# ratschlab/SVGP-VAE

Hardware: AMD Instinct MI355X
Metric: SVGPVAE train steps/sec, rotated MNIST (N=4050, M=32, L=16) (higher is better)
Workload: dtype f64; 1 GPU; BASELINE configs[1]: rotated-MNIST SVGPVAE_Hensman, m=32 inducing, L=16, GPLVM dim 8, batch 256 per GPU, N_train=4050, GECO + clip_qs, float64; global_batch=256, rows_per_gpu=256, launch=eager phases (faster of hipGraph replay / eager phases in an untimed probe), parallelism=dp1, single_stat_block=0

## Files before the change

svgp-vae_amd/csrc/vae_dev.hpp:

```cpp
#pragma once
#include "common.hpp"

namespace svgp_vae {

#define VAE_NT 512
#define VAE_SCRATCH 4096

typedef double d4v_t __attribute__((ext_vector_type(4)));

template <int NTAP, bool TW, bool ELU_BIAS, int CI, int CO, int NT = VAE_NT>
__device__ __forceinline__ void gg_fwd(const real* in, int Hi, int Wi, int Hs, int Ws, int sy, int sx,
                                       const int (&oy)[NTAP], const int (&ox)[NTAP], const int (&woff)[NTAP],
                                       const real* W, int ldw, const real* bias, real* out, int Wo, int osy, int osx,
                                       int ooy, int oox) {
    constexpr int KQ = (CI + 3) / 4;
    const int lane = threadIdx.x & 63, wave = threadIdx.x >> 6, nwave = NT >> 6, r = lane & 15, q = lane >> 4;
    const int NP = Hs * Ws, ngrp = (NP + 15) >> 4;
    real breg[NTAP * KQ];
#pragma unroll
    for (int t = 0; t < NTAP; ++t)
#pragma unroll
        for (int kq = 0; kq < KQ; ++kq) {
            const int c = kq * 4 + q, cc = c < CI ? c : CI - 1, rc = r < CO ? r : CO - 1;
            const real v = W[woff[t] + (TW ? rc * ldw + cc : cc * ldw + rc)];
// ... 96 lines not shown
    static __device__ void fwd(const real* in, const real* w, const real* bias, real* out) {
        if constexpr (CIN == 1) {
            for (int it = threadIdx.x; it < NPIX * COUT; it += NT) {
                const int co = it % COUT, p = it / COUT, y = p / HOUT, x = p % HOUT;
                real acc = bias[co];
#pragma unroll
                for (int ky = 0; ky < 3; ++ky)
#pragma unroll
                    for (int kx = 0; kx < 3; ++kx) acc += in[(2 * y + ky) * HS + 2 * x + kx] * w[(ky * 3 + kx) * COUT + co];
                out[it] = elu_f(acc);
            }
            return;
        }
        const int oy[9] = {0, 0, 0, 1, 1, 1, 2, 2, 2}, ox[9] = {0, 1, 2, 0, 1, 2, 0, 1, 2};
        int wo[9];
#pragma unroll
        for (int t = 0; t < 9; ++t) wo[t] = t * CIN * COUT;
        gg_fwd<9, false, true, CIN, COUT, NT>(in, HS, HS, HOUT, HOUT, 2, 2, oy, ox, wo, w, COUT, bias, out, HOUT, 1, 1, 0, 0);
    }

    static __device__ void bwd_data(const real* dpre, const real* w, real* din) {
        {
            const int oy[4] = {0, 0, -1, -1}, ox[4] = {0, -1, 0, -1};
            const int wo[4] = {(0 * 3 + 0) * CIN * COUT, (0 * 3 + 2) * CIN * COUT, (2 * 3 + 0) * CIN * COUT, (2 * 3 + 2) * CIN * COUT};
            gg_fwd<4, true, false, COUT, CIN, NT>(dpre, HOUT, HOUT, (HS + 1) / 2, (HS + 1) / 2, 1, 1, oy, ox, wo, w, COUT, nullptr,
                                              din, HS, 2, 2, 0, 0);
        }
        {
            const int oy[2] = {0, -1}, ox[2] = {0, 0};
            const int wo[2] = {(0 * 3 + 1) * CIN * COUT, (2 * 3 + 1) * CIN * COUT};
            gg_fwd<2, true, false, COUT, CIN, NT>(dpre, HOUT, HOUT, (HS + 1) / 2, HS / 2, 1, 1, oy, ox, wo, w, COUT, nullptr, din,
                                              HS, 2, 2, 0, 1);
        }
        {
            const int oy[2] = {0, 0}, ox[2] = {0, -1};
            const int wo[2] = {(1 * 3 + 0) * CIN * COUT, (1 * 3 + 2) * CIN * COUT};
            gg_fwd<2, true, false, COUT, CIN, NT>(dpre, HOUT, HOUT, HS / 2, (HS + 1) / 2, 1, 1, oy, ox, wo, w, COUT, nullptr, din,
                                              HS, 2, 2, 1, 0);
        }
        {
            const int oy[1] = {0}, ox[1] = {0};
            const int wo[1] = {(1 * 3 + 1) * CIN * COUT};
            gg_fwd<1, true, false, COUT, CIN, NT>(dpre, HOUT, HOUT, HS / 2, HS / 2, 1, 1, oy, ox, wo, w, COUT, nullptr, din, HS, 2,
                                              2, 1, 1);
        }
    }

    static __device__ void bwd_weight(const real* in, const real* dpre, real* gw, real* gb, real* scratch) {
        if constexpr (CIN == 1) {
            constexpr int NO = 9 * COUT, NCH = NT / NO;
            static_assert(NCH >= 1 && NO * NCH <= VAE_SCRATCH, "chunk layout");
            const int o = threadIdx.x % NO, ch = threadIdx.x / NO, t = o / COUT, co = o % COUT, ky = t / 3, kx = t % 3;
            if (ch < NCH) {
                real acc = 0;
                for (int p = ch; p < NPIX; p += NCH) {
                    const int y = p / HOUT, x = p % HOUT;
                    acc += in[(2 * y + ky) * HS + 2 * x + kx] * dpre[p * COUT + co];
                }
                scratch[ch * NO + o] = acc;
            }
            __syncthreads();
            if (threadIdx.x < NO) {
                real tsum = 0;
#pragma unroll
                for (int c = 0; c < NCH; ++c) tsum += scratch[c * NO + threadIdx.x];
                gw[threadIdx.x] += tsum;
            }
            __syncthreads();
        } else {
            auto tapfn = [](int t) { return TapP{t / 3, t % 3, t * CIN * COUT, 0, 0}; };
            gg_wgrad<9, CIN, COUT, NT>(in, HS, HS, HOUT, HOUT, 2, 2, tapfn, dpre, HOUT, 1, 1, gw);
        }
        bias_grad<NPIX, COUT, NT>(dpre, gb, scratch);
    }
};

template <int HS, int PAD, int CIN, int COUT, int NT = VAE_NT>
struct UpConv3 {
    static constexpr int HOUT = 2 * HS - 2 + 2 * PAD;
    static constexpr int NPIX = HOUT * HOUT;
    static constexpr int NWE = 16 * CIN * COUT;
    static constexpr int NW = 9 * CIN * COUT;
    static constexpr int COG = (COUT % 2 == 0) ? 2 : 1;
    static constexpr int NCG = COUT / COG;
    static constexpr int CIG = (CIN % 2 == 0) ? 2 : 1;
    static constexpr int NIG = CIN / CIG;
    static __device__ __forceinline__ int T(int pi, int k) { return (k + pi >= 2) ? 1 : 0; }

    static __device__ void build_weff(const real* w, real* We) {
        for (int e = threadIdx.x; e < NWE; e += NT) {
            const int co = e % COUT, ci = (e / COUT) % CIN, tap = (e / (COUT * CIN)) % 4, cls = e / (COUT * CIN * 4);
            const int ty = tap >> 1, tx = tap & 1, py = cls >> 1, px = cls & 1;
            real s = 0;
#pragma unroll
            for (int ky = 0; ky < 3; ++ky)
#pragma unroll
                for (int kx = 0; kx < 3; ++kx)
                    if (T(py, ky) == ty && T(px, kx) == tx) s += w[((ky * 3 + kx) * CIN + ci) * COUT + co];
            We[e] = s;
        }
    }
    static __device__ void fold_grad(const real* gWe, real* gw) {
        for (int e = threadIdx.x; e < NW; e += NT) {
            const int co = e % COUT, ci = (e / COUT) % CIN, kx = (e / (COUT * CIN)) % 3, ky = e / (COUT * CIN * 3);
            real s = 0;
#pragma unroll
            for (int py = 0; py < 2; ++py)
#pragma unroll
                for (int px = 0; px < 2; ++px)
                    s += gWe[(((py * 2 + px) * 4 + T(py, ky) * 2 + T(px, kx)) * CIN + ci) * COUT + co];
            gw[e] = s;
        }
    }

    template <bool ROLL = false>
    static __device__ void fwd_valu(const real* in, const real* We, const real* bias, real* out) {
        constexpr int TAP_UNROLL = ROLL ? 1 : 2;
        for (int it = threadIdx.x; it < NPIX * NCG; it += NT) {
            const int cg = it % NCG, p = it / NCG, x = p % HOUT, y = p / HOUT;
            const int by = y - PAD, bx = x - PAD, py = by & 1, px = bx & 1, Y = by >> 1, X = bx >> 1;
            real acc[COG];
#pragma unroll
            for (int g = 0; g < COG; ++g) acc[g] = bias[cg * COG + g];
            const real* wc = We + ((py * 2 + px) * 4) * CIN * COUT + cg * COG;
#pragma unroll TAP_UNROLL
            for (int ty = 0; ty < 2; ++ty) {
                const int sy = Y + ty;
                const bool vy = (unsigned)sy < (unsigned)HS;
#pragma unroll TAP_UNROLL
                for (int tx = 0; tx < 2; ++tx) {
                    const int sx = X + tx;
                    const bool valid = vy && ((unsigned)sx < (unsigned)HS);
                    const real* src = in + (valid ? (sy * HS + sx) * CIN : 0);
                    const real* wk = wc + (ty * 2 + tx) * CIN * COUT;
#pragma unroll
                    for (int ci = 0; ci < CIN; ++ci) {
                        const real a = valid ? src[ci] : real(0);
#pragma unroll
                        for (int g = 0; g < COG; ++g) acc[g] += a * wk[ci * COUT + g];
                    }
                }
            }
#pragma unroll
            for (int g = 0; g < COG; ++g) out[p * COUT + cg * COG + g] = elu_f(acc[g]);
        }
    }

    static __device__ void bwd_data_valu(const real* dpre, const real* We, real* din) {
        for (int it = threadIdx.x; it < HS * HS * NIG; it += NT) {
            const int ig = it % NIG, ps = it / NIG, Xs = ps % HS, Ys = ps / HS;
            real acc[CIG];
#pragma unroll
            for (int g = 0; g < CIG; ++g) acc[g] = 0;
#pragma unroll 1
            for (int cy = 0; cy < 4; ++cy) {
                const int py = cy >> 1, ty = cy & 1;
                const int y = 2 * (Ys - ty) + py + PAD;
                const bool vy = (unsigned)y < (unsigned)HOUT;
#pragma unroll
                for (int cx = 0; cx < 4; ++cx) {
                    const int px = cx >> 1, tx = cx & 1;
                    const int x = 2 * (Xs - tx) + px + PAD;
                    const bool valid = vy && ((unsigned)x < (unsigned)HOUT);
                    const real* dp = dpre + (valid ? (y * HOUT + x) * COUT : 0);
                    const real* wk = We + (((py * 2 + px) * 4 + ty * 2 + tx) * CIN + ig * CIG) * COUT;
#pragma unroll
                    for (int co = 0; co < COUT; ++co) {
                        const real d = valid ? dp[co] : real(0);
#pragma unroll
                        for (int g = 0; g < CIG; ++g) acc[g] += d * wk[g * COUT + co];
                    }
                }
            }
#pragma unroll
            for (int g = 0; g < CIG; ++g) din[ps * CIN + ig * CIG + g] = acc[g];
        }
    }

    static __device__ void bwd_weight_valu(const real* in, const real* dpre, real* gWe, real* gb, real* scratch) {
        constexpr int NTC = 16 * CIN;
        constexpr int NCH0 = NT / NTC, NCH1 = VAE_SCRATCH / NWE;
        constexpr int NCH = NCH0 < NCH1 ? (NCH0 < 1 ? 1 : NCH0) : NCH1;
        constexpr int NG = HS + 1;
        const int tc = threadIdx.x % NTC, chunk = threadIdx.x / NTC;
        if (chunk < NCH) {
            const int ci = tc % CIN, tap = (tc / CIN) % 4, cls = tc / (CIN * 4);
            const int ty = tap >> 1, tx = tap & 1, py = cls >> 1, px = cls & 1;
            real acc[COUT];
#pragma unroll
            for (int co = 0; co < COUT; ++co) acc[co] = 0;
#pragma unroll 2
            for (int idx = chunk; idx < NG * NG; idx += NCH) {
                const int Y = idx / NG - 1, X = idx % NG - 1;
                const int y = 2 * Y + py + PAD, x = 2 * X + px + PAD, sy = Y + ty, sx = X + tx;
                const bool valid = ((unsigned)y < (unsigned)HOUT) && ((unsigned)x < (unsigned)HOUT) &&
                                   ((unsigned)sy < (unsigned)HS) && ((unsigned)sx < (unsigned)HS);
                const real a = valid ? in[(sy * HS + sx) * CIN + ci] : real(0);
                const real* dp = dpre + (valid ? (y * HOUT + x) * COUT : 0);
#pragma unroll
                for (int co = 0; co < COUT; ++co) acc[co] += a * dp[co];
            }
#pragma unroll
            for (int co = 0; co < COUT; ++co) scratch[chunk * NWE + tc * COUT + co] = acc[co];
        }
        __syncthreads();
        for (int widx = threadIdx.x; widx < NWE; widx += NT) {
            real s = 0;
#pragma unroll
            for (int c = 0; c < NCH; ++c) s += scratch[c * NWE + widx];
            gWe[widx] += s;
        }
        __syncthreads();
        constexpr int BCH = 32;
        if (threadIdx.x < BCH * COUT) {
            const int co = threadIdx.x % COUT, chunk2 = threadIdx.x / COUT;
            real s = 0;
            for (int p = chunk2; p < NPIX; p += BCH) s += dpre[p * COUT + co];
            scratch[threadIdx.x] = s;
        }
        __syncthreads();
        if (threadIdx.x < COUT) {
            real t = 0;
#pragma unroll
            for (int c = 0; c < BCH; ++c) t += scratch[c * COUT + threadIdx.x];
            gb[threadIdx.x] += t;
        }
        __syncthreads();
    }

    static __device__ void bwd_data_mfma(const real* dpre, const real* We, real* din) {
        int oy[16], ox[16], wo[16];
#pragma unroll
        for (int t = 0; t < 16; ++t) {
            const int py = (t >> 3) & 1, ty = (t >> 2) & 1, px = (t >> 1) & 1, tx = t & 1;
            oy[t] = py + PAD - 2 * ty;
            ox[t] = px + PAD - 2 * tx;
            wo[t] = ((py * 2 + px) * 4 + ty * 2 + tx) * CIN * COUT;
        }
        gg_fwd<16, true, false, COUT, CIN, NT>(dpre, HOUT, HOUT, HS, HS, 2, 2, oy, ox, wo, We, COUT, nullptr, din, HS, 1, 1, 0, 0);
    }

    static __device__ void bwd_weight_mfma(const real* in, const real* dpre, real* gWe, real* gb, real* scratch) {
        if (COUT >= 2) {
            auto tapfn = [](int t) {
                const int opy = (t >> 3) & 1, opx = (t >> 2) & 1, ty = (t >> 1) & 1, tx = t & 1;
                const int by = opy - PAD, bx = opx - PAD, py = by & 1, px = bx & 1;
                return TapP{(by - py) / 2 + ty, (bx - px) / 2 + tx, ((py * 2 + px) * 4 + ty * 2 + tx) * CIN * COUT, opy, opx};
            };
            gg_wgrad<16, CIN, COUT, NT>(in, HS, HS, HOUT / 2, HOUT / 2, 1, 1, tapfn, dpre, HOUT, 2, 2, gWe);
        } else {
            constexpr int NCH = NT / 16;
            constexpr int NG = HS + 1;
            const int ct = threadIdx.x & 15, chunk = threadIdx.x >> 4;
            const int cls = ct >> 2, tap = ct & 3, ty = tap >> 1, tx = tap & 1, py = cls >> 1, px = cls & 1;
            real acc[CIN];
#pragma unroll
            for (int ci = 0; ci < CIN; ++ci) acc[ci] = 0;
            for (int idx = chunk; idx < NG * NG; idx += NCH) {
                const int Y = idx / NG - 1, X = idx % NG - 1;
                const int y = 2 * Y + py + PAD, x = 2 * X + px + PAD, sy = Y + ty, sx = X + tx;
                const bool valid = ((unsigned)y < (unsigned)HOUT) && ((unsigned)x < (unsigned)HOUT) &&
                                   ((unsigned)sy < (unsigned)HS) && ((unsigned)sx < (unsigned)HS);
                const real d = valid ? dpre[y * HOUT + x] : real(0);
                const real* ip = in + (valid ? (sy * HS + sx) * CIN : 0);
#pragma unroll
                for (int ci = 0; ci < CIN; ++ci) acc[ci] += ip[ci] * d;
            }
#pragma unroll
            for (int ci = 0; ci < CIN; ++ci) scratch[chunk * (16 * CIN) + ct * CIN + ci] = acc[ci];
            __syncthreads();
            for (int widx = threadIdx.x; widx < 16 * CIN; widx += NT) {
                real s = 0;
#pragma unroll 8
                for (int c = 0; c < NCH; ++c) s += scratch[c * (16 * CIN) + widx];
                gWe[widx] += s;
            }
        }
        __syncthreads();
        bias_grad<NPIX, COUT, NT>(dpre, gb, scratch);
    }
};

template <int NT> using UpC1T = UpConv3<4, 1, 8, 8, NT>;
using UpC1 = UpC1T<VAE_NT>;
template <int NT> using UpC2T = UpConv3<8, 0, 8, 8, NT>;
using UpC2 = UpC2T<VAE_NT>;
template <int NT> using UpC3T = UpConv3<14, 1, 8, 1, NT>;
using UpC3 = UpC3T<VAE_NT>;
#define DEC_NWE 2176
static_assert(UpC1::NWE + UpC2::NWE + UpC3::NWE == DEC_NWE, "effective weights of the three up-convolutions");

using EncC1 = Conv3<28, 1, 0, 2, 1, 8, 13>;
using EncC2 = Conv3<13, 1, 0, 2, 8, 8, 6>;
using EncC3 = Conv3<6, 1, 0, 2, 8, 8, 2>;

__device__ __forceinline__ void lds_copy_in(real* dst, const real* __restrict__ src, int n) {
    for (int i = threadIdx.x; i < n; i += blockDim.x) dst[i] = src[i];
}
__device__ __forceinline__ void lds_copy_out(real* __restrict__ dst, const real* src, int n) {
    for (int i = threadIdx.x; i < n; i += blockDim.x) dst[i] = src[i];
}
__device__ __forceinline__ void lds_zero(real* dst, int n) {
    for (int i = threadIdx.x; i < n; i += blockDim.x) dst[i] = 0;
}

struct EncOff { int c1w, c1b, c2w, c2b, c3w, c3b, dw, db, n; };
struct DecOff { int dw, db, c1w, c1b, c2w, c2b, c3w, c3b, n; };

__device__ __host__ inline EncOff enc_off(int L) {
    EncOff o; int p = 0;
    o.c1w = p; p += 72; o.c1b = p; p += 8; o.c2w = p; p += 576; o.c2b = p; p += 8;
    o.c3w = p; p += 576; o.c3b = p; p += 8; o.dw = p; p += 32 * 2 * L; o.db = p; p += 2 * L; o.n = p;
    return o;
}
__device__ __host__ inline DecOff dec_off(int L) {
    DecOff o; int p = 0;
    o.dw = p; p += L * 128; o.db = p; p += 128; o.c1w = p; p += 576; o.c1b = p; p += 8;
    o.c2w = p; p += 576; o.c2b = p; p += 8; o.c3w = p; p += 72; o.c3b = p; p += 1; o.n = p;
    return o;
}


struct DecWgradArgs {
    int b, L, geco, n_slots, n_types;
    real inv_bglobal;
    const real* state; const real* images; const real* z; const real* h0; const real* a1; const real* a2; const real* recon;
    const real* d2; const real* d1; const real* dh0;
    real* part;
};
__host__ __device__ constexpr int dec_wgrad_mask(int n_types, int ty) { return n_types == 1 ? 7 : n_types == 2 ? (ty == 0 ? 1 : 6) : (1 << ty); }
__host__ __device__ constexpr int dec_wgrad_lds_mask(int nt, int L, int mask) {
    return ((mask & 1) ? 1568 + 784 + 128 : 0) + ((mask & 2) ? 512 + 1568 + 1024 : 0) +
           ((mask & 4) ? 128 + 512 + 128 + 64 + 1024 + L * 128 + 128 : 0) + 32 + ((mask & 3) ? (nt <= 256 ? 2048 : 4096) : 256);
}
__host__ __device__ constexpr int dec_wgrad_lds(int nt, int L, int n_types) {
    int mx = 0;
    for (int ty = 0; ty < n_types; ++ty) {
        const int v = dec_wgrad_lds_mask(nt, L, dec_wgrad_mask(n_types, ty));
        mx = v > mx ? v : mx;
    }
    return mx;
}

template <int NT>
__device__ __forceinline__ void decoder_wgrad_rider(const DecWgradArgs& a, int rider, real* smem) {
    static_assert(NT >= 256 && NT <= 512, "bias / chunk layouts are sized for 256..512 threads");
    const DecOff od = dec_off(a.L);
    const int tyo = rider / a.n_slots, slot = rider - tyo * a.n_slots;
    const int ty = a.n_types == 3 ? (tyo == 0 ? 1 : tyo == 1 ? 0 : 2) : a.n_types == 2 ? 1 - tyo : 0;
    const int mask = dec_wgrad_mask(a.n_types, ty);
    const int ndense = a.L * 128;
    real* p = smem;
    auto take = [&](int n) { real* r = p; p += n; return r; };
    real *a2 = nullptr, *d3 = nullptr, *gWe3 = nullptr, *a1 = nullptr, *d2 = nullptr, *gWe2 = nullptr, *h0 = nullptr, *d1 = nullptr,
         *dh0 = nullptr, *z = nullptr, *gWe1 = nullptr, *dacc = nullptr;
    if (mask & 1) { a2 = take(1568); d3 = take(784); gWe3 = take(128); }
    if (mask & 2) { a1 = take(512); d2 = take(1568); gWe2 = take(1024); }
    if (mask & 4) { h0 = take(128); d1 = take(512); dh0 = take(128); z = take(64); gWe1 = take(1024); dacc = take(ndense + 128); }
    real* gb = take(32);
    real* scratch = p;
    if (mask & 1) for (int i = threadIdx.x; i < 128; i += NT) gWe3[i] = 0;
    if (mask & 2) for (int i = threadIdx.x; i < 1024; i += NT) gWe2[i] = 0;
    if (mask & 4) for (int i = threadIdx.x; i < 1024 + ndense + 128; i += NT) gWe1[i] = 0;
    if (threadIdx.x < 32) gb[threadIdx.x] = 0;
    const real gscale = (a.geco ? a.state[SVGP_ST_LAGRANGE] * a.inv_bglobal : real(1)) / real(784);
    for (int n = slot; n < a.b; n += a.n_slots) {
        __syncthreads();
        if (mask & 1) {
            for (int i = threadIdx.x; i < 784; i += NT) {
                const real o = a.recon[(size_t)n * 784 + i];
                d3[i] = real(2) * gscale * (o - a.images[(size_t)n * 784 + i]) * elu_grad_from_out(o);
            }
            for (int i = threadIdx.x; i < 1568; i += NT) a2[i] = a.a2[(size_t)n * 1568 + i];
        }
        if (mask & 2) {
            for (int i = threadIdx.x; i < 1568; i += NT) d2[i] = a.d2[(size_t)n * 1568 + i];
            for (int i = threadIdx.x; i < 512; i += NT) a1[i] = a.a1[(size_t)n * 512 + i];
        }
        if (mask & 4) {
            for (int i = threadIdx.x; i < 512; i += NT) d1[i] = a.d1[(size_t)n * 512 + i];
            if (threadIdx.x < 128) { h0[threadIdx.x] = a.h0[(size_t)n * 128 + threadIdx.x]; dh0[threadIdx.x] = a.dh0[(size_t)n * 128 + threadIdx.x]; }
            if ((int)threadIdx.x < a.L) z[threadIdx.x] = a.z[(size_t)n * a.L + threadIdx.x];
        }
        __syncthreads();
        if (mask & 1) UpC3T<NT>::bwd_weight_mfma(a2, d3, gWe3, gb + 16, scratch);
        if (mask & 2) UpC2T<NT>::bwd_weight_valu(a1, d2, gWe2, gb + 8, scratch);
        if (mask & 4) {
            UpC1T<NT>::bwd_weight_mfma(h0, d1, gWe1, gb, scratch);
            for (int o = threadIdx.x; o < ndense; o += NT) dacc[o] += z[o >> 7] * dh0[o & 127];
            if (threadIdx.x < 128) dacc[ndense + threadIdx.x] += dh0[threadIdx.x];
        }
    }
    __syncthreads();
    real* part = a.part + (size_t)slot * od.n;
    if (mask & 1) {
        UpC3T<NT>::fold_grad(gWe3, part + od.c3w);
        if (threadIdx.x == 0) part[od.c3b] = gb[16];
    }
    if (mask & 2) {
        UpC2T<NT>::fold_grad(gWe2, part + od.c2w);
        if (threadIdx.x < 8) part[od.c2b + threadIdx.x] = gb[8 + threadIdx.x];
    }
    if (mask & 4) {
        UpC1T<NT>::fold_grad(gWe1, part + od.c1w);
        if (threadIdx.x < 8) part[od.c1b + threadIdx.x] = gb[threadIdx.x];
        for (int o = threadIdx.x; o < ndense; o += NT) part[od.dw + o] = dacc[o];
        if (threadIdx.x < 128) part[od.db + threadIdx.x] = dacc[ndense + threadIdx.x];
    }
}

struct DecBwdDataArgs {
    int b, L, geco;
    real inv_bglobal;
    const real* state; const real* th_dec; const real* images; const real* a1g; const real* a2g; const real* recon;
    real* d2g; real* d1g; real* dh0g; real* zbar;
    const real* weff;
};
__host__ __device__ constexpr int dec_bwd_data_lds(int L, int n_dec, bool pre) {
    return L * 128 + DEC_NWE + 512 + 1568 + 784 + 1568 + 512 + 128 + (pre ? 0 : n_dec - L * 128 - 128);
}
template <bool PRE>
__device__ __forceinline__ void decoder_bwd_data_images(const DecBwdDataArgs& a, int first, int stride, real* smem) {
    const DecOff od = dec_off(a.L);
    real* w = smem;
    real* We1 = w + a.L * 128;
    real* We2 = We1 + UpC1::NWE;
    real* We3 = We2 + UpC2::NWE;
    real* a1 = We3 + UpC3::NWE;
    real* a2 = a1 + 512;
    real* d3 = a2 + 1568;
    real* d2 = d3 + 784;
    real* d1 = d2 + 1568;
    real* dh0 = d1 + 512;
    real* raw = dh0 + 128;
    lds_copy_in(w, a.th_dec + od.dw, a.L * 128);
    if (PRE) {
        lds_copy_in(We1, a.weff, DEC_NWE);
    } else {
        lds_copy_in(raw, a.th_dec + od.c1w, od.n - od.c1w);
        __syncthreads();
        UpC1::build_weff(raw, We1);
        UpC2::build_weff(raw + (od.c2w - od.c1w), We2);
        UpC3::build_weff(raw + (od.c3w - od.c1w), We3);
    }
    const real gscale = (a.geco ? a.state[SVGP_ST_LAGRANGE] * a.inv_bglobal : real(1)) / real(784);
    for (int n = first; n < a.b; n += stride) {
        __syncthreads();
        lds_copy_in(a1, a.a1g + (size_t)n * 512, 512);
        lds_copy_in(a2, a.a2g + (size_t)n * 1568, 1568);
        for (int i = threadIdx.x; i < 784; i += blockDim.x) {
            const real o = a.recon[(size_t)n * 784 + i];
            d3[i] = real(2) * gscale * (o - a.images[(size_t)n * 784 + i]) * elu_grad_from_out(o);
        }
        __syncthreads();
        UpC3::bwd_data_valu(d3, We3, d2);
        __syncthreads();
        for (int i = threadIdx.x; i < 1568; i += blockDim.x) {
            const real v = d2[i] * elu_grad_from_out(a2[i]);
            d2[i] = v;
            a.d2g[(size_t)n * 1568 + i] = v;
        }
        svgp_lds_barrier();
        UpC2::bwd_data_mfma(d2, We2, d1);
        svgp_lds_barrier();
        for (int i = threadIdx.x; i < 512; i += blockDim.x) {
            const real v = d1[i] * elu_grad_from_out(a1[i]);
            d1[i] = v;
            a.d1g[(size_t)n * 512 + i] = v;
        }
        svgp_lds_barrier();
        UpC1::bwd_data_mfma(d1, We1, dh0);
        svgp_lds_barrier();
        if (threadIdx.x < 128) a.dh0g[(size_t)n * 128 + threadIdx.x] = dh0[threadIdx.x];
        {
            const int i = threadIdx.x >> 3, part8 = threadIdx.x & 7;
            real acc = 0;
            if (i < a.L)
                for (int j = part8; j < 128; j += 8) acc += dh0[j] * w[i * 128 + j];
            acc += __shfl_xor(acc, 1, 64);
            acc += __shfl_xor(acc, 2, 64);
            acc += __shfl_xor(acc, 4, 64);
            if (i < a.L && part8 == 0) a.zbar[(size_t)n * a.L + i] = acc;
        }
    }
}

struct DecFwdBwdArgs {
    int b, L, geco;
    real inv_bglobal;
    const real* state; const real* th_dec; const real* images; const real* zg; const real* weff;
    real* h0g; real* a1g; real* a2g; real* recon; real* part_sums;
    real* d2g; real* d1g; real* dh0g; real* zbar;
};
__host__ __device__ constexpr int dec_fwd_bwd_lds(int L) {
    return L * 128 + 128 + 32 + DEC_NWE + 64 + 128 + 512 + 1568 + 784 + 1568 + 512 + 128 + 16;
}
__device__ __forceinline__ void decoder_fwd_bwd_data_images(const DecFwdBwdArgs& a, int first, int stride, real* smem) {
    const DecOff od = dec_off(a.L);
    real* w = smem;
    real* db = w + a.L * 128;
    real* cb = db + 128;
    real* We1 = cb + 32;
    real* We2 = We1 + UpC1::NWE;
    real* We3 = We2 + UpC2::NWE;
    real* z = We3 + UpC3::NWE;
    real* h0 = z + 64;
    real* a1 = h0 + 128;
    real* a2 = a1 + 512;
    real* d3 = a2 + 1568;
    real* d2 = d3 + 784;
    real* d1 = d2 + 1568;
    real* dh0 = d1 + 512;
    real* red = dh0 + 128;
    const int t = threadIdx.x;
    const real lag = a.geco ? a.state[SVGP_ST_LAGRANGE] : real(0);
    real zr = t < a.L ? a.zg[(size_t)first * a.L + t] : real(0);
    real px0 = a.images[(size_t)first * 784 + t];
    real px1 = t + VAE_NT < 784 ? a.images[(size_t)first * 784 + t + VAE_NT] : real(0);
    lds_copy_in(w, a.th_dec + od.dw, a.L * 128 + 128);
    if (t < 8) { cb[t] = a.th_dec[od.c1b + t]; cb[8 + t] = a.th_dec[od.c2b + t]; }
    if (t == 0) cb[16] = a.th_dec[od.c3b];
    lds_copy_in(We1, a.weff, DEC_NWE);
    const real gscale = (a.geco ? lag * a.inv_bglobal : real(1)) / real(784);
    real sq = 0;
    for (int n = first; n < a.b; n += stride) {
        __syncthreads();
        if (t < a.L) z[t] = zr;
        __syncthreads();
        if (t < 128) {
            real acc = db[t];
            for (int i = 0; i < a.L; ++i) acc += z[i] * w[i * 128 + t];
            h0[t] = acc;
        }
        __syncthreads();
        UpC1::fwd_valu<true>(h0, We1, cb, a1);
        __syncthreads();
        UpC2::fwd_valu<true>(a1, We2, cb + 8, a2);
        __syncthreads();
        UpC3::fwd_valu<true>(a2, We3, cb + 16, d3);
        __syncthreads();
        lds_copy_out(a.h0g + (size_t)n * 128, h0, 128);
        lds_copy_out(a.a1g + (size_t)n * 512, a1, 512);
        lds_copy_out(a.a2g + (size_t)n * 1568, a2, 1568);
        {
            const real o = d3[t];
            a.recon[(size_t)n * 784 + t] = o;
            const real df = px0 - o;
            sq += df * df;
            d3[t] = real(2) * gscale * (o - px0) * elu_grad_from_out(o);
            if (t + VAE_NT < 784) {
                const real o1 = d3[t + VAE_NT];
                a.recon[(size_t)n * 784 + t + VAE_NT] = o1;
                const real df1 = px1 - o1;
                sq += df1 * df1;
                d3[t + VAE_NT] = real(2) * gscale * (o1 - px1) * elu_grad_from_out(o1);
            }
        }
        {
            const int nn = n + stride;
            if (nn < a.b) {
                zr = t < a.L ? a.zg[(size_t)nn * a.L + t] : real(0);
                px0 = a.images[(size_t)nn * 784 + t];
                px1 = t + VAE_NT < 784 ? a.images[(size_t)nn * 784 + t + VAE_NT] : real(0);
            }
        }
        __syncthreads();
        UpC3::bwd_data_valu(d3, We3, d2);
        __syncthreads();
        for (int i = t; i < 1568; i += VAE_NT) {
            const real v = d2[i] * elu_grad_from_out(a2[i]);
            d2[i] = v;
            a.d2g[(size_t)n * 1568 + i] = v;
        }
        svgp_lds_barrier();
        UpC2::bwd_data_mfma(d2, We2, d1);
        svgp_lds_barrier();
        for (int i = t; i < 512; i += VAE_NT) {
            const real v = d1[i] * elu_grad_from_out(a1[i]);
            d1[i] = v;
            a.d1g[(size_t)n * 512 + i] = v;
        }
        svgp_lds_barrier();
        UpC1::bwd_data_mfma(d1, We1, dh0);
        svgp_lds_barrier();
        if (t < 128) a.dh0g[(size_t)n * 128 + t] = dh0[t];
        {
            const int i = t >> 3, part8 = t & 7;
            real acc = 0;
            if (i < a.L)
                for (int j = part8; j < 128; j += 8) acc += dh0[j] * w[i * 128 + j];
            acc += __shfl_xor(acc, 1, 64);
            acc += __shfl_xor(acc, 2, 64);
            acc += __shfl_xor(acc, 4, 64);
            if (i < a.L && part8 == 0) a.zbar[(size_t)n * a.L + i] = acc;
        }
    }
    const real tot = block_sum(sq, red);
    if (t == 0) a.part_sums[first * 4 + 2] = tot;
}

struct EncBwdArgs {
    int b, L, clip;
    const real* th_enc; const real* images; const real* a1g; const real* a2g; const real* a3g; const real* var_raw;
    const real* ybar; const real* s2bar;
    real* part;
};
#define ENC_BWD_SCRATCH 512
__host__ __device__ constexpr int enc_bwd_lds(int n_enc) {
    return 2 * n_enc + 784 + 1352 + 288 + 32 + 1352 + 288 + 32 + 128 + ENC_BWD_SCRATCH;
}

template <int NT>
__device__ __forceinline__ void encoder_bwd_images(const EncBwdArgs& a, int first, int stride, real* smem) {
    const int L = a.L;
    const EncOff eo = enc_off(L);
    real* w = smem;
    real* g = w + eo.n;
    real* img = g + eo.n;
    real* a1 = img + 784;
    real* a2 = a1 + 1352;
    real* a3 = a2 + 288;
    real* d1 = a3 + 32;
    real* d2 = d1 + 1352;
    real* d3 = d2 + 288;
    real* dout = d3 + 32;
    real* scratch = dout + 128;
    using C1 = Conv3<28, 1, 0, 2, 1, 8, 13, NT>;
    using C2 = Conv3<13, 1, 0, 2, 8, 8, 6, NT>;
    using C3 = Conv3<6, 1, 0, 2, 8, 8, 2, NT>;
    static_assert(72 * (NT / 72) <= ENC_BWD_SCRATCH, "first-layer chunk scratch");
    lds_copy_in(w, a.th_enc, eo.n);
    lds_zero(g, eo.n);
    const int twoL = 2 * L;
    for (int n = first; n < a.b; n += stride) {
        __syncthreads();
        lds_copy_in(img, a.images + (size_t)n * 784, 784);
        lds_copy_in(a1, a.a1g + (size_t)n * 1352, 1352);
        lds_copy_in(a2, a.a2g + (size_t)n * 288, 288);
        lds_copy_in(a3, a.a3g + (size_t)n * 32, 32);
        for (int j = threadIdx.x; j < twoL; j += NT) {
            real dj;
            if (j < L) {
                dj = a.ybar[(size_t)n * L + j];
            } else {
                const real vr = a.var_raw[(size_t)n * L + j - L];
                const real sb = a.s2bar[(size_t)n * L + j - L];
                const bool pass = !a.clip || (vr >= 1e-3 && vr <= 10.0);
                dj = pass ? sb * vr : real(0);
            }
            dout[j] = dj;
        }
        __syncthreads();
        for (int o = threadIdx.x; o < 32 * twoL; o += NT) g[eo.dw + o] += a3[o / twoL] * dout[o % twoL];
        for (int j = threadIdx.x; j < twoL; j += NT) g[eo.db + j] += dout[j];
        if (threadIdx.x < 32) {
            real acc = 0;
            for (int j = 0; j < twoL; ++j) acc += dout[j] * w[eo.dw + threadIdx.x * twoL + j];
            d3[threadIdx.x] = acc * elu_grad_from_out(a3[threadIdx.x]);
        }
        __syncthreads();
        C3::bwd_weight(a2, d3, g + eo.c3w, g + eo.c3b, scratch);
        C3::bwd_data(d3, w + eo.c3w, d2);
        __syncthreads();
        for (int i = threadIdx.x; i < 288; i += NT) d2[i] *= elu_grad_from_out(a2[i]);
        __syncthreads();
        C2::bwd_weight(a1, d2, g + eo.c2w, g + eo.c2b, scratch);
        C2::bwd_data(d2, w + eo.c2w, d1);
        __syncthreads();
        for (int i = threadIdx.x; i < 1352; i += NT) d1[i] *= elu_grad_from_out(a1[i]);
        __syncthreads();
        C1::bwd_weight(img, d1, g + eo.c1w, g + eo.c1b, scratch);
    }
    __syncthreads();
    lds_copy_out(a.part + (size_t)first * eo.n, g, eo.n);
}

}

svgp_vae::DecWgradArgs svgp_make_dec_wgrad_args(const svgp_mnist_cfg* c, const svgp_mnist_ws_layout& wl, const double* images,
                                                double* ws, const double* state, int n_types);
svgp_vae::DecBwdDataArgs svgp_make_dec_bwd_data_args(const svgp_mnist_cfg* c, const svgp_mnist_ws_layout& wl, const double* theta,
                                                     const double* images, double* ws, const double* state);
svgp_vae::EncBwdArgs svgp_make_enc_bwd_args(const svgp_mnist_cfg* c, const svgp_mnist_ws_layout& wl, const double* theta,
                                            const double* images, double* ws);
```

svgp-vae_amd/csrc/vae_mnist.hip:

```cpp
#include <cstdlib>

#include "common.hpp"
#include "vae_dev.hpp"

namespace {

using namespace svgp_vae;

__global__ __launch_bounds__(VAE_NT) void k_encoder_fwd(int b, int L, int clip, const real* __restrict__ th_enc,
                                                            const real* __restrict__ images, real* __restrict__ a1g,
                                                            real* __restrict__ a2g, real* __restrict__ a3g,
                                                            real* __restrict__ mu, real* __restrict__ var_raw,
                                                            real* __restrict__ var, int n_img_blocks, SvgpKernArgs ka,
                                                            real* __restrict__ Kmm, real* __restrict__ Knm,
                                                            real* __restrict__ knn, int n_km_blocks,
                                                            const real* __restrict__ th_dec, real* __restrict__ weff) {
    extern __shared__ __align__(16) real smem[];
    if ((int)blockIdx.x >= n_img_blocks + n_km_blocks) {
        const DecOff od = dec_off(L);
        UpC1::build_weff(th_dec + od.c1w, weff);
        UpC2::build_weff(th_dec + od.c2w, weff + UpC1::NWE);
        UpC3::build_weff(th_dec + od.c3w, weff + UpC1::NWE + UpC2::NWE);
        return;
    }
    if ((int)blockIdx.x >= n_img_blocks) {
        svgp_km_fwd_element(ka, (long long)(blockIdx.x - n_img_blocks) * blockDim.x + threadIdx.x, Kmm, Knm, knn);
        return;
    }
    const EncOff eo = enc_off(L);
    real* w = smem;
    real* img = w + eo.n;
    real* a1 = img + 784;
    real* a2 = a1 + 1352;
    real* a3 = a2 + 288;
    lds_copy_in(w, th_enc, eo.n);
    for (int n = blockIdx.x; n < b; n += n_img_blocks) {
        __syncthreads();
        lds_copy_in(img, images + (size_t)n * 784, 784);
        __syncthreads();
        EncC1::fwd(img, w + eo.c1w, w + eo.c1b, a1);
        __syncthreads();
        EncC2::fwd(a1, w + eo.c2w, w + eo.c2b, a2);
        __syncthreads();
        EncC3::fwd(a2, w + eo.c3w, w + eo.c3b, a3);
        __syncthreads();
        lds_copy_out(a1g + (size_t)n * 1352, a1, 1352);
        lds_copy_out(a2g + (size_t)n * 288, a2, 288);
        lds_copy_out(a3g + (size_t)n * 32, a3, 32);
        const int twoL = 2 * L;
        for (int j = threadIdx.x; j < twoL; j += blockDim.x) {
            real acc = w[eo.db + j];
            for (int i = 0; i < 32; ++i) acc += a3[i] * w[eo.dw + i * twoL + j];
            if (j < L) {
                mu[(size_t)n * L + j] = acc;
            } else {
                const real vr = exp(acc);
                var_raw[(size_t)n * L + j - L] = vr;
                var[(size_t)n * L + j - L] = clip ? fmin(fmax(vr, 1e-3), 10.0) : vr;
            }
        }
    }
}

__global__ __launch_bounds__(VAE_NT) void k_encoder_bwd(EncBwdArgs a) {
    extern __shared__ __align__(16) real smem[];
    encoder_bwd_images<VAE_NT>(a, blockIdx.x, gridDim.x, smem);
}

template <bool PRE>
__global__ __launch_bounds__(VAE_NT) void k_decoder_fwd(int b, int L, const real* __restrict__ th_dec,
                                                            const real* __restrict__ images,
                                                            const real* __restrict__ zg, real* __restrict__ h0g,
                                                            real* __restrict__ a1g, real* __restrict__ a2g,
                                                            real* __restrict__ recon, real* __restrict__ part_sums,
                                                            const real* __restrict__ weff) {
    extern __shared__ __align__(16) real smem[];
    const DecOff od = dec_off(L);
    real* w = smem;
    real* z = w + od.n;
    real* h0 = z + 64;
    real* a1 = h0 + 128;
    real* a2 = a1 + 512;
    real* out = a2 + 1568;
    real* red = out + 784;
    real* We1 = red + 16;
    real* We2 = We1 + UpC1::NWE;
    real* We3 = We2 + UpC2::NWE;
    lds_copy_in(w, th_dec, od.n);
    if (PRE) {
        lds_copy_in(We1, weff, DEC_NWE);
    } else {
        __syncthreads();
        UpC1::build_weff(w + od.c1w, We1);
        UpC2::build_weff(w + od.c2w, We2);
        UpC3::build_weff(w + od.c3w, We3);
    }
    real sq = 0;
    for (int n = blockIdx.x; n < b; n += gridDim.x) {
        __syncthreads();
        lds_copy_in(z, zg + (size_t)n * L, L);
        __syncthreads();
        if (threadIdx.x < 128) {
            real acc = w[od.db + threadIdx.x];
            for (int i = 0; i < L; ++i) acc += z[i] * w[od.dw + i * 128 + threadIdx.x];
            h0[threadIdx.x] = acc;
        }
        __syncthreads();
        UpC1::fwd_valu(h0, We1, w + od.c1b, a1);
        __syncthreads();
        UpC2::fwd_valu(a1, We2, w + od.c2b, a2);
        __syncthreads();
        UpC3::fwd_valu(a2, We3, w + od.c3b, out);
        __syncthreads();
        lds_copy_out(h0g + (size_t)n * 128, h0, 128);
        lds_copy_out(a1g + (size_t)n * 512, a1, 512);
        lds_copy_out(a2g + (size_t)n * 1568, a2, 1568);
        for (int i = threadIdx.x; i < 784; i += blockDim.x) {
            const real o = out[i];
            recon[(size_t)n * 784 + i] = o;
            const real df = images[(size_t)n * 784 + i] - o;
            sq += df * df;
        }
    }
    const real tot = block_sum(sq, red);
    if (threadIdx.x == 0) part_sums[blockIdx.x * 4 + 2] = tot;
}

__global__ __launch_bounds__(VAE_NT) void k_decoder_bwd(int b, int L, int geco, real inv_bglobal,
                                                            const real* __restrict__ state,
                                                            const real* __restrict__ th_dec,
                                                            const real* __restrict__ images,
                                                            const real* __restrict__ zg, const real* __restrict__ h0g,
                                                            const real* __restrict__ a1g, const real* __restrict__ a2g,
                                                            const real* __restrict__ recon, real* __restrict__ zbar,
                                                            real* __restrict__ part) {
    extern __shared__ __align__(16) real smem[];
    const DecOff od = dec_off(L);
    real* w = smem;
    real* g = w + L * 128;
    real* We1 = g + od.n;
    real* We2 = We1 + UpC1::NWE;
    real* We3 = We2 + UpC2::NWE;
    real* gWe1 = We3 + UpC3::NWE;
    real* gWe2 = gWe1 + UpC1::NWE;
    real* gWe3 = gWe2 + UpC2::NWE;
    real* z = gWe3 + UpC3::NWE;
    real* h0 = z + 64;
    real* a1 = h0 + 128;
    real* a2 = a1 + 512;
    real* d3 = a2 + 1568;
    real* d2 = d3 + 784;
    real* d1 = d2 + 1568;
    real* dh0 = d1 + 512;
    real* scratch = dh0 + 128;
    lds_copy_in(w, th_dec + od.dw, L * 128);
    lds_zero(g, od.n);
    lds_zero(gWe1, DEC_NWE);
    lds_copy_in(scratch, th_dec + od.c1w, od.n - od.c1w);
    __syncthreads();
    UpC1::build_weff(scratch, We1);
    UpC2::build_weff(scratch + (od.c2w - od.c1w), We2);
    UpC3::build_weff(scratch + (od.c3w - od.c1w), We3);
    const real gscale = (geco ? state[SVGP_ST_LAGRANGE] * inv_bglobal : real(1)) / real(784);
    for (int n = blockIdx.x; n < b; n += gridDim.x) {
        __syncthreads();
        lds_copy_in(z, zg + (size_t)n * L, L);
        lds_copy_in(h0, h0g + (size_t)n * 128, 128);
        lds_copy_in(a1, a1g + (size_t)n * 512, 512);
        lds_copy_in(a2, a2g + (size_t)n * 1568, 1568);
        for (int i = threadIdx.x; i < 784; i += blockDim.x) {
            const real o = recon[(size_t)n * 784 + i];
            d3[i] = real(2) * gscale * (o - images[(size_t)n * 784 + i]) * elu_grad_from_out(o);
        }
        __syncthreads();
        UpC3::bwd_weight_mfma(a2, d3, gWe3, g + od.c3b, scratch);
        UpC3::bwd_data_valu(d3, We3, d2);
        __syncthreads();
        for (int i = threadIdx.x; i < 1568; i += blockDim.x) d2[i] *= elu_grad_from_out(a2[i]);
        __syncthreads();
        UpC2::bwd_weight_valu(a1, d2, gWe2, g + od.c2b, scratch);
        UpC2::bwd_data_mfma(d2, We2, d1);
        __syncthreads();
        for (int i = threadIdx.x; i < 512; i += blockDim.x) d1[i] *= elu_grad_from_out(a1[i]);
        __syncthreads();
        UpC1::bwd_weight_mfma(h0, d1, gWe1, g + od.c1b, scratch);
        UpC1::bwd_data_mfma(d1, We1, dh0);
        __syncthreads();
        for (int o = threadIdx.x; o < L * 128; o += blockDim.x) g[od.dw + o] += z[o / 128] * dh0[o % 128];
        if (threadIdx.x < 128) g[od.db + threadIdx.x] += dh0[threadIdx.x];
        {
            const int i = threadIdx.x >> 3, part8 = threadIdx.x & 7;
            real acc = 0;
            if (i < L)
                for (int j = part8; j < 128; j += 8) acc += dh0[j] * w[i * 128 + j];
            acc += __shfl_xor(acc, 1, 64);
            acc += __shfl_xor(acc, 2, 64);
            acc += __shfl_xor(acc, 4, 64);
            if (i < L && part8 == 0) zbar[(size_t)n * L + i] = acc;
        }
    }
    __syncthreads();
    UpC1::fold_grad(gWe1, g + od.c1w);
    UpC2::fold_grad(gWe2, g + od.c2w);
    UpC3::fold_grad(gWe3, g + od.c3w);
    __syncthreads();
    lds_copy_out(part + (size_t)blockIdx.x * od.n, g, od.n);
}

template <bool PRE>
__global__ __launch_bounds__(VAE_NT) void k_decoder_bwd_data(DecBwdDataArgs a) {
    extern __shared__ __align__(16) real smem[];
    decoder_bwd_data_images<PRE>(a, blockIdx.x, gridDim.x, smem);
}

template <int NT>
__global__ __launch_bounds__(NT) void k_decoder_bwd_weights(DecWgradArgs a) {
    extern __shared__ __align__(16) real smem[];
    decoder_wgrad_rider<NT>(a, blockIdx.x, smem);
}

struct KmScatter {
    int n_blocks, M, n_obj, n_gp_part, train_gp, train_ov;
    const real* aux; const real* d_on; const real* part_gp;
    real* d_ov; real* d_ls; real* d_amp;
};

__global__ __launch_bounds__(SVGP_BLOCK) void k_grad_reduce(int n_part, int n_enc, int n_dec, int nb_enc, int nb_dec,
                                                            int n_post, int b, const real* __restrict__ part_enc,
                                                            const real* __restrict__ part_dec,
                                                            const real* __restrict__ part_sums,
                                                            const real* __restrict__ tit_rowsum,
                                                            real* __restrict__ grad, real* __restrict__ sums,
                                                            KmScatter ks, int blk0) {
    __shared__ real s[16][17];
    __shared__ real red[16];
    const int bid = (int)blockIdx.x + blk0;
    if (bid > nb_enc + nb_dec) {
        svgp_km_scatter_block(bid - (nb_enc + nb_dec + 1), ks.n_blocks, b, ks.M, ks.n_obj, ks.aux, ks.n_gp_part,
                              ks.train_gp, ks.train_ov, ks.d_on, ks.part_gp, ks.d_ov, ks.d_ls, ks.d_amp);
        return;
    }
    if (bid == nb_enc + nb_dec) {
        real l3 = 0, ce = 0, sq = 0;
        for (int i = threadIdx.x; i < n_part; i += blockDim.x) sq += part_sums[i * 4 + 2];
        const real* pp = part_sums + (size_t)n_part * 4;
        for (int i = threadIdx.x; i < n_post; i += blockDim.x) { l3 += pp[i * 2]; ce += pp[i * 2 + 1]; }
        l3 = block_sum(l3, red);
        ce = block_sum(ce, red);
        sq = block_sum(sq, red);
        if (threadIdx.x == 0) {
            sums[0] = l3; sums[1] = ce; sums[2] = sq; sums[3] = (real)b;
            sums[4] = tit_rowsum ? *tit_rowsum : real(0);
            sums[5] = 0; sums[6] = 0; sums[7] = 0;
        }
        return;
    }
    const bool enc = bid < nb_enc;
    const int n = enc ? n_enc : n_dec, blk = enc ? bid : bid - nb_enc;
    const real* part = enc ? part_enc : part_dec;
    real* out = enc ? grad : grad + n_enc;
    const int il = threadIdx.x & 15, ch = threadIdx.x >> 4;
    const int i = blk * 16 + il;
    real acc = 0;
    if (i < n) {
#pragma unroll 4
        for (int wq = ch; wq < n_part; wq += 16) acc += part[(size_t)wq * n + i];
    }
    s[ch][il] = acc;
    __syncthreads();
    if (ch == 0 && i < n) {
        real t = 0;
#pragma unroll
        for (int c = 0; c < 16; ++c) t += s[c][il];
        out[i] = t;
    }
}

template <typename F>
int set_dyn_lds(F kernel, size_t bytes) {
    SVGP_CHECK_HIP(hipFuncSetAttribute(reinterpret_cast<const void*>(kernel),
                                       hipFuncAttributeMaxDynamicSharedMemorySize, (int)bytes));
    return SVGP_OK;
}

}

#define GET_LAYOUTS()                                          \
    svgp_mnist_param_layout pl;                                \
    svgp_mnist_ws_layout wl;                                   \
    {                                                          \
        int rc_ = svgp_mnist_param_layout_get(c, &pl);         \
        if (rc_) return rc_;                                   \
        rc_ = svgp_mnist_ws_layout_get(c, &wl);                \
        if (rc_) return rc_;                                   \
    }

static int encoder_fwd_impl(const svgp_mnist_cfg* c, const double* theta, const double* images, const double* aux,
                            double* ws, void* stream) {
    GET_LAYOUTS();
    SVGP_REQUIRE(theta && images && ws, SVGP_ERR_INVALID, "NULL device pointer");
    const size_t lds = (size_t)(pl.n_enc + 784 + 1352 + 288 + 32) * sizeof(real);
    int rc = set_dyn_lds(k_encoder_fwd, lds);
    if (rc) return rc;
    const int n_img = svgp_n_part(c);
    SvgpKernArgs ka;
    memset(&ka, 0, sizeof(ka));
    int n_km = 0;
    if (aux) {
        ka = svgp_make_kern_args(c, pl, theta, aux);
        const long long nel = (long long)c->b * c->m + (long long)c->m * c->m + c->b;
        n_km = (int)((nel + VAE_NT - 1) / VAE_NT);
    }
    hipLaunchKernelGGL(k_encoder_fwd, dim3(n_img + n_km + (aux ? 1 : 0)), dim3(VAE_NT), lds, (hipStream_t)stream, c->b, c->L,
                       c->clip_qs, theta, images, ws + wl.enc_a1, ws + wl.enc_a2, ws + wl.enc_a3, ws + wl.qnet_mu,
                       ws + wl.qnet_var_raw, ws + wl.qnet_var, n_img, ka, ws + wl.K, ws + wl.Kn, ws + wl.knn, n_km,
                       theta + pl.n_enc, ws + wl.dec_weff);
    SVGP_LAUNCH_CHECK();
    return SVGP_OK;
}

extern "C" int svgp_mnist_encoder_fwd(const svgp_mnist_cfg* c, const double* theta, const double* images, double* ws,
                                      void* stream) {
    return encoder_fwd_impl(c, theta, images, nullptr, ws, stream);
}

extern "C" int svgp_mnist_encoder_kernel_matrix_fwd(const svgp_mnist_cfg* c, const double* theta, const double* images,
                                                    const double* aux, double* ws, void* stream) {
    SVGP_REQUIRE(aux, SVGP_ERR_INVALID, "NULL device pointer");
    return encoder_fwd_impl(c, theta, images, aux, ws, stream);
}

extern "C" int svgp_mnist_encoder_bwd(const svgp_mnist_cfg* c, const double* theta, const double* images, double* ws,
                                      void* stream) {
    GET_LAYOUTS();
    SVGP_REQUIRE(theta && images && ws, SVGP_ERR_INVALID, "NULL device pointer");
    const size_t lds = (size_t)enc_bwd_lds((int)pl.n_enc) * sizeof(real);
    int rc = set_dyn_lds(k_encoder_bwd, lds);
    if (rc) return rc;
    hipLaunchKernelGGL(k_encoder_bwd, dim3(svgp_n_part(c)), dim3(VAE_NT), lds, (hipStream_t)stream,
                       svgp_make_enc_bwd_args(c, wl, theta, images, ws));
    SVGP_LAUNCH_CHECK();
    return SVGP_OK;
}

static int decoder_fwd_impl(const svgp_mnist_cfg* c, const double* theta, const double* images, double* ws, bool pre, void* stream) {
    GET_LAYOUTS();
    SVGP_REQUIRE(theta && images && ws, SVGP_ERR_INVALID, "NULL device pointer");
    const int64_t n_dec = pl.n_vae - pl.n_enc;
    const size_t lds = (size_t)(n_dec + 64 + 128 + 512 + 1568 + 784 + 16 + DEC_NWE) * sizeof(real);
    int rc = pre ? set_dyn_lds(k_decoder_fwd<true>, lds) : set_dyn_lds(k_decoder_fwd<false>, lds);
    if (rc) return rc;
#define DEC_FWD_ARGS c->b, c->L, theta + pl.n_enc, images, ws + wl.z, ws + wl.dec_h0, ws + wl.dec_a1, ws + wl.dec_a2, ws + wl.recon, \
                     ws + wl.part_sums, ws + wl.dec_weff
    if (pre) hipLaunchKernelGGL(k_decoder_fwd<true>, dim3(svgp_n_part(c)), dim3(VAE_NT), lds, (hipStream_t)stream, DEC_FWD_ARGS);
    else hipLaunchKernelGGL(k_decoder_fwd<false>, dim3(svgp_n_part(c)), dim3(VAE_NT), lds, (hipStream_t)stream, DEC_FWD_ARGS);
#undef DEC_FWD_ARGS
    SVGP_LAUNCH_CHECK();
    return SVGP_OK;
}
extern "C" int svgp_mnist_decoder_fwd(const svgp_mnist_cfg* c, const double* theta, const double* images, double* ws,
                                      void* stream) {
    return decoder_fwd_impl(c, theta, images, ws, false, stream);
}
extern "C" int svgp_mnist_decoder_fwd_pre(const svgp_mnist_cfg* c, const double* theta, const double* images, double* ws,
                                          void* stream) {
    return decoder_fwd_impl(c, theta, images, ws, true, stream);
}

extern "C" int svgp_mnist_decoder_bwd(const svgp_mnist_cfg* c, const double* theta, const double* images, double* ws,
                                      const double* state, void* stream) {
    GET_LAYOUTS();
    SVGP_REQUIRE(theta && images && ws && state, SVGP_ERR_INVALID, "NULL device pointer");
    const int64_t n_dec = pl.n_vae - pl.n_enc;
    const size_t lds = (size_t)(c->L * 128 + n_dec + 2 * DEC_NWE + 64 + 128 + 512 + 1568 + 784 + 1568 + 512 + 128 + VAE_SCRATCH) * sizeof(real);
    if (lds > SVGP_LDS_MAX_BYTES) {
        int rc = svgp_mnist_decoder_bwd_data(c, theta, images, ws, state, stream);
        if (rc) return rc;
        return svgp_mnist_decoder_bwd_weights(c, images, ws, state, 256, 3, stream);
    }
    int rc = set_dyn_lds(k_decoder_bwd, lds);
    if (rc) return rc;
    hipLaunchKernelGGL(k_decoder_bwd, dim3(svgp_n_part(c)), dim3(VAE_NT), lds, (hipStream_t)stream, c->b, c->L,
                       c->geco, 1.0 / (double)c->b_global, state, theta + pl.n_enc, images, ws + wl.z, ws + wl.dec_h0,
                       ws + wl.dec_a1, ws + wl.dec_a2, ws + wl.recon, ws + wl.zbar, ws + wl.part_dec);
    SVGP_LAUNCH_CHECK();
    return SVGP_OK;
}

svgp_vae::DecBwdDataArgs svgp_make_dec_bwd_data_args(const svgp_mnist_cfg* c, const svgp_mnist_ws_layout& wl, const double* theta,
                                                     const double* images, double* ws, const double* state) {
    svgp_mnist_param_layout pl;
    svgp_mnist_param_layout_get(c, &pl);
    DecBwdDataArgs a;
    a.b = c->b; a.L = c->L; a.geco = c->geco; a.inv_bglobal = 1.0 / (double)c->b_global;
    a.state = state; a.th_dec = theta + pl.n_enc; a.images = images; a.a1g = ws + wl.dec_a1; a.a2g = ws + wl.dec_a2;
    a.recon = ws + wl.recon; a.d2g = ws + wl.dec_d2; a.d1g = ws + wl.dec_d1; a.dh0g = ws + wl.dec_dh0; a.zbar = ws + wl.zbar;
    a.weff = ws + wl.dec_weff;
    return a;
}
static int decoder_bwd_data_impl(const svgp_mnist_cfg* c, const double* theta, const double* images, double* ws,
                                 const double* state, bool pre, void* stream) {
    GET_LAYOUTS();
    SVGP_REQUIRE(theta && images && ws && state, SVGP_ERR_INVALID, "NULL device pointer");
    const int64_t n_dec = pl.n_vae - pl.n_enc;
    const size_t lds = (size_t)dec_bwd_data_lds(c->L, (int)n_dec, pre) * sizeof(real);
    int rc = pre ? set_dyn_lds(k_decoder_bwd_data<true>, lds) : set_dyn_lds(k_decoder_bwd_data<false>, lds);
    if (rc) return rc;
    const DecBwdDataArgs a = svgp_make_dec_bwd_data_args(c, wl, theta, images, ws, state);
    if (pre) hipLaunchKernelGGL(k_decoder_bwd_data<true>, dim3(svgp_n_part(c)), dim3(VAE_NT), lds, (hipStream_t)stream, a);
    else hipLaunchKernelGGL(k_decoder_bwd_data<false>, dim3(svgp_n_part(c)), dim3(VAE_NT), lds, (hipStream_t)stream, a);
    SVGP_LAUNCH_CHECK();
    return SVGP_OK;
}
extern "C" int svgp_mnist_decoder_bwd_data(const svgp_mnist_cfg* c, const double* theta, const double* images, double* ws,
                                           const double* state, void* stream) {
    return decoder_bwd_data_impl(c, theta, images, ws, state, false, stream);
}
extern "C" int svgp_mnist_decoder_bwd_data_pre(const svgp_mnist_cfg* c, const double* theta, const double* images, double* ws,
                                               const double* state, void* stream) {
    return decoder_bwd_data_impl(c, theta, images, ws, state, true, stream);
}

svgp_vae::EncBwdArgs svgp_make_enc_bwd_args(const svgp_mnist_cfg* c, const svgp_mnist_ws_layout& wl, const double* theta,
                                            const double* images, double* ws) {
// ... 74 lines not shown
```

Measured before the change: 7294 steps/s (256-row batches, whole job).

## Stage per-image global loads through registers to overlap with weight staging

Replaces the strided global-to-LDS copy loops in the decoder forward, decoder backward-data and encoder backward kernels with register-staged loads. The per-image activations and pixels are issued into registers early, before the weight copy or at the top of each image iteration, and committed to LDS afterwards, so more global loads are in flight at once. The weight copy is batched into chunks of eight loads per thread before the stores. The aim is to hide global memory latency in these latency-bound per-image loops, at the cost of higher register pressure (several thousand doubles spread across 512 threads) and possible occupancy loss.

```diff
diff --git a/svgp-vae_amd/csrc/vae_dev.hpp b/svgp-vae_amd/csrc/vae_dev.hpp
--- a/svgp-vae_amd/csrc/vae_dev.hpp
+++ b/svgp-vae_amd/csrc/vae_dev.hpp
@@ -422,6 +422,48 @@
 }
 __device__ __forceinline__ void lds_zero(real* dst, int n) {
     for (int i = threadIdx.x; i < n; i += blockDim.x) dst[i] = 0;
+}
+
+template <int N, int NT>
+__device__ __forceinline__ int stage_spare() { return N >= NT ? (int)threadIdx.x : min((int)threadIdx.x, N - 1); }
+template <int N, int NT>
+struct StageRegs {
+    static constexpr int C = (N + NT - 1) / NT;
+    real v[C];
+};
+template <int N, int NT>
+__device__ __forceinline__ StageRegs<N, NT> stage_issue(const real* __restrict__ src) {
+    StageRegs<N, NT> r;
+#pragma unroll
+    for (int k = 0; k < StageRegs<N, NT>::C; ++k) {
+        const int i = (int)threadIdx.x + k * NT;
+        r.v[k] = src[(k + 1) * NT <= N || i < N ? i : stage_spare<N, NT>()];
+    }
+    return r;
+}
+template <int N, int NT>
+__device__ __forceinline__ void stage_commit(real* dst, const StageRegs<N, NT>& r) {
+#pragma unroll
+    for (int k = 0; k < StageRegs<N, NT>::C; ++k) {
+        const int i = (int)threadIdx.x + k * NT;
+        if ((k + 1) * NT <= N || i < N) dst[i] = r.v[k];
+    }
+}
+template <int NT, int CH>
+__device__ __forceinline__ void stage_chunk(real* dst, const real* __restrict__ src, int n, int c0) {
+    const int base = c0 + (int)threadIdx.x, spare = min(base, n - 1);
+    real r[CH];
+#pragma unroll
+    for (int k = 0; k < CH; ++k) r[k] = src[base + k * NT < n ? base + k * NT : spare];
+    __atomic_signal_fence(__ATOMIC_SEQ_CST);
+#pragma unroll
+    for (int k = 0; k < CH; ++k)
+        if (base + k * NT < n) dst[base + k * NT] = r[k];
+}
+template <int NT, int CH = 8>
+__device__ __forceinline__ void stage_copy(real* dst, const real* __restrict__ src, int n) {
+    stage_chunk<NT, CH>(dst, src, n, 0);
+    for (int c0 = CH * NT; c0 < n; c0 += CH * NT) stage_chunk<NT, CH>(dst, src, n, c0);
 }
 
 struct EncOff { int c1w, c1b, c2w, c2b, c3w, c3b, dw, db, n; };
@@ -553,11 +595,20 @@
     real* d1 = d2 + 1568;
     real* dh0 = d1 + 512;
     real* raw = dh0 + 128;
-    lds_copy_in(w, a.th_dec + od.dw, a.L * 128);
+    const int nf = first < a.b ? first : a.b - 1;
+    auto ra1 = stage_issue<512, VAE_NT>(a.a1g + (size_t)nf * 512);
+    auto ra2 = stage_issue<1568, VAE_NT>(a.a2g + (size_t)nf * 1568);
+    auto rrec = stage_issue<784, VAE_NT>(a.recon + (size_t)nf * 784);
+    auto rpx = stage_issue<784, VAE_NT>(a.images + (size_t)nf * 784);
     if (PRE) {
-        lds_copy_in(We1, a.weff, DEC_NWE);
+        const auto rwe = stage_issue<DEC_NWE, VAE_NT>(a.weff);
+        stage_copy<VAE_NT>(w, a.th_dec + od.dw, a.L * 128);
+        stage_commit<DEC_NWE, VAE_NT>(We1, rwe);
     } else {
-        lds_copy_in(raw, a.th_dec + od.c1w, od.n - od.c1w);
+        constexpr int NRAW = 576 + 8 + 576 + 8 + 72 + 1;
+        const auto rraw = stage_issue<NRAW, VAE_NT>(a.th_dec + od.c1w);
+        stage_copy<VAE_NT>(w, a.th_dec + od.dw, a.L * 128);
+        stage_commit<NRAW, VAE_NT>(raw, rraw);
         __syncthreads();
         UpC1::build_weff(raw, We1);
         UpC2::build_weff(raw + (od.c2w - od.c1w), We2);
@@ -566,11 +617,19 @@
     const real gscale = (a.geco ? a.state[SVGP_ST_LAGRANGE] * a.inv_bglobal : real(1)) / real(784);
     for (int n = first; n < a.b; n += stride) {
         __syncthreads();
-        lds_copy_in(a1, a.a1g + (size_t)n * 512, 512);
-        lds_copy_in(a2, a.a2g + (size_t)n * 1568, 1568);
-        for (int i = threadIdx.x; i < 784; i += blockDim.x) {
-            const real o = a.recon[(size_t)n * 784 + i];
-            d3[i] = real(2) * gscale * (o - a.images[(size_t)n * 784 + i]) * elu_grad_from_out(o);
+        if (n != first) {
+            ra1 = stage_issue<512, VAE_NT>(a.a1g + (size_t)n * 512);
+            ra2 = stage_issue<1568, VAE_NT>(a.a2g + (size_t)n * 1568);
+            rrec = stage_issue<784, VAE_NT>(a.recon + (size_t)n * 784);
+            rpx = stage_issue<784, VAE_NT>(a.images + (size_t)n * 784);
+        }
+        stage_commit<512, VAE_NT>(a1, ra1);
+        stage_commit<1568, VAE_NT>(a2, ra2);
+#pragma unroll
+        for (int k = 0; k < 2; ++k) {
+            const int i = (int)threadIdx.x + k * VAE_NT;
+            const real o = rrec.v[k];
+            if (i < 784) d3[i] = real(2) * gscale * (o - rpx.v[k]) * elu_grad_from_out(o);
         }
         __syncthreads();
         UpC3::bwd_data_valu(d3, We3, d2);
@@ -749,26 +808,33 @@
     using C2 = Conv3<13, 1, 0, 2, 8, 8, 6, NT>;
     using C3 = Conv3<6, 1, 0, 2, 8, 8, 2, NT>;
     static_assert(72 * (NT / 72) <= ENC_BWD_SCRATCH, "first-layer chunk scratch");
-    lds_copy_in(w, a.th_enc, eo.n);
-    lds_zero(g, eo.n);
-    const int twoL = 2 * L;
+    static_assert(NT >= 128, "thread j stages dout[j], j < 2L <= 128");
+    const int twoL = 2 * L, t = threadIdx.x;
+    const int jy = t < L ? t : L - 1, jv = t < L ? 0 : t < twoL ? t - L : L - 1;
+    StageRegs<784, NT> rimg; StageRegs<1352, NT> ra1; StageRegs<288, NT> ra2; StageRegs<32, NT> ra3;
+    real ryb, rvr, rsb;
+    auto issue = [&](int n) {
+        rimg = stage_issue<784, NT>(a.images + (size_t)n * 784);
+        ra1 = stage_issue<1352, NT>(a.a1g + (size_t)n * 1352);
+        ra2 = stage_issue<288, NT>(a.a2g + (size_t)n * 288);
+        ra3 = stage_issue<32, NT>(a.a3g + (size_t)n * 32);
+        ryb = a.ybar[(size_t)n * L + jy];
+        rvr = a.var_raw[(size_t)n * L + jv];
+        rsb = a.s2bar[(size_t)n * L + jv];
+    };
+    issue(first < a.b ? first : a.b - 1);
+    stage_copy<NT>(w, a.th_enc, eo.n);
+    for (int i = t; i < eo.n; i += NT) g[i] = 0;
     for (int n = first; n < a.b; n += stride) {
         __syncthreads();
-        lds_copy_in(img, a.images + (size_t)n * 784, 784);
-        lds_copy_in(a1, a.a1g + (size_t)n * 1352, 1352);
-        lds_copy_in(a2, a.a2g + (size_t)n * 288, 288);
-        lds_copy_in(a3, a.a3g + (size_t)n * 32, 32);
-        for (int j = threadIdx.x; j < twoL; j += NT) {
-            real dj;
-            if (j < L) {
-                dj = a.ybar[(size_t)n * L + j];
-            } else {
-                const real vr = a.var_raw[(size_t)n * L + j - L];
-                const real sb = a.s2bar[(size_t)n * L + j - L];
-                const bool pass = !a.clip || (vr >= 1e-3 && vr <= 10.0);
-                dj = pass ? sb * vr : real(0);
-            }
-            dout[j] = dj;
+        if (n != first) issue(n);
+        stage_commit<784, NT>(img, rimg);
+        stage_commit<1352, NT>(a1, ra1);
+        stage_commit<288, NT>(a2, ra2);
+        stage_commit<32, NT>(a3, ra3);
+        if (t < twoL) {
+            const bool pass = !a.clip || (rvr >= 1e-3 && rvr <= 10.0);
+            dout[t] = t < L ? ryb : pass ? rsb * rvr : real(0);
         }
         __syncthreads();
         for (int o = threadIdx.x; o < 32 * twoL; o += NT) g[eo.dw + o] += a3[o / twoL] * dout[o % twoL];
diff --git a/svgp-vae_amd/csrc/vae_mnist.hip b/svgp-vae_amd/csrc/vae_mnist.hip
--- a/svgp-vae_amd/csrc/vae_mnist.hip
+++ b/svgp-vae_amd/csrc/vae_mnist.hip
@@ -86,10 +86,14 @@
     real* We1 = red + 16;
     real* We2 = We1 + UpC1::NWE;
     real* We3 = We2 + UpC2::NWE;
-    lds_copy_in(w, th_dec, od.n);
+    const int t = threadIdx.x, lz = t < L ? t : L - 1;
+    real zr = zg[(size_t)min((int)blockIdx.x, b - 1) * L + lz];
     if (PRE) {
-        lds_copy_in(We1, weff, DEC_NWE);
+        const auto rwe = stage_issue<DEC_NWE, VAE_NT>(weff);
+        stage_copy<VAE_NT>(w, th_dec, od.n);
+        stage_commit<DEC_NWE, VAE_NT>(We1, rwe);
     } else {
+        stage_copy<VAE_NT>(w, th_dec, od.n);
         __syncthreads();
         UpC1::build_weff(w + od.c1w, We1);
         UpC2::build_weff(w + od.c2w, We2);
@@ -98,7 +102,9 @@
     real sq = 0;
     for (int n = blockIdx.x; n < b; n += gridDim.x) {
         __syncthreads();
-        lds_copy_in(z, zg + (size_t)n * L, L);
+        if (t < L) z[t] = zr;
+        const auto px = stage_issue<784, VAE_NT>(images + (size_t)n * 784);
+        if (n + (int)gridDim.x < b) zr = zg[(size_t)(n + gridDim.x) * L + lz];
         __syncthreads();
         if (threadIdx.x < 128) {
             real acc = w[od.db + threadIdx.x];
@@ -115,11 +121,15 @@
         lds_copy_out(h0g + (size_t)n * 128, h0, 128);
         lds_copy_out(a1g + (size_t)n * 512, a1, 512);
         lds_copy_out(a2g + (size_t)n * 1568, a2, 1568);
-        for (int i = threadIdx.x; i < 784; i += blockDim.x) {
-            const real o = out[i];
-            recon[(size_t)n * 784 + i] = o;
-            const real df = images[(size_t)n * 784 + i] - o;
-            sq += df * df;
+#pragma unroll
+        for (int k = 0; k < 2; ++k) {
+            const int i = t + k * VAE_NT;
+            if (i < 784) {
+                const real o = out[i];
+                recon[(size_t)n * 784 + i] = o;
+                const real df = px.v[k] - o;
+                sq += df * df;
+            }
         }
     }
     const real tot = block_sum(sq, red);
```

Result: faster. 7437 steps/s (256-row batches, whole job), median of 6 (+2.0%).
